# RuanJohn/Mava

Measured on AMD Instinct MI355X. Metric: env-steps/sec (whole node), ff_mappo RWARE tiny-4ag, higher is better.
Workload: dtype f32 via 2 x f16 split operands on the MFMA (3 products, f32 accumulate); 1 GPU; ff_mappo RWARE tiny-4ag-shaped synthetic obs, 4096 envs/GPU (update_batch_size=1 x num_envs=4096), rollout_length=128, ppo_epochs=4, num_minibatches=2, agents=4, obs=70/264, actions=5, one step = one PPO update = 524288 env-steps per GPU; parallelism=dp1

## Files before the change

### include/mava_hip.h

```cpp
#ifndef MAVA_HIP_H
#define MAVA_HIP_H

#include <stddef.h>
#include <stdint.h>

#ifdef __cplusplus
extern "C" {
#endif

typedef struct ihipStream_t* mava_stream_t;

const char* mava_last_error(void);
int mava_abi_version(void);

typedef struct mava_ctx mava_ctx;
enum {
  MAVA_CTX_MATMUL_MODE = 0,
  MAVA_CTX_CRITIC_AGGREGATION = 1,
  MAVA_CTX_GAE_VARIANT = 2,
  MAVA_CTX_POLICY_VARIANT = 3,
  MAVA_CTX_H2_LAUNCHES = 4,
  MAVA_CTX_TRAIN_VARIANT = 5,
  MAVA_CTX_W8_LAUNCHES = 6,
  MAVA_CTX_W1_SPLIT_FRESH = 7
};
int mava_ctx_create(mava_ctx** out);
int mava_ctx_destroy(mava_ctx* ctx);
int mava_ctx_set(mava_ctx* ctx, int key, long value);
int mava_ctx_get(const mava_ctx* ctx, int key, long* value);

int mava_gae_f32(const mava_ctx* ctx, const float* reward, const float* value, const uint8_t* done,
                 const float* last_val, const uint8_t* last_done, int T, int N, float gamma,
                 float lambda, float* adv, float* tgt, mava_stream_t s);

int mava_permutation_i32(long n, uint64_t seed, uint64_t counter, int32_t* out, mava_stream_t s);

int mava_clip_adam(float* p, const float* g, float* m, float* v, int32_t* count,
                   const int* seg_off, const float* seg_lr, int n_seg, float grad_scale,
                   float max_norm, int decay, int steps_per_update, int num_updates, float b1,
// ... 244 lines not shown
```

### mava_amd/_lib.py

```python
from __future__ import annotations

import ctypes as C
import os
from typing import Optional

import torch

_HERE = os.path.dirname(os.path.abspath(__file__))
LIB_PATH = os.environ.get("MAVA_LIB_PATH") or os.path.join(_HERE, "libmavahip.so")

_lib: Optional[C.CDLL] = None


class MavaHipError(RuntimeError):
    pass


vp = C.c_void_p
i32 = C.c_int
u32 = C.c_uint32
u64 = C.c_uint64
f32 = C.c_float
lng = C.c_long

# ... 83 lines not shown
                f"{LIB_PATH} is missing: build it with `python -m mava_amd.build` "
                "(hipcc --offload-arch=gfx950). There is no CPU fallback."
            )
        _lib = C.CDLL(LIB_PATH)
        _lib.mava_last_error.restype = C.c_char_p
        _lib.mava_last_error.argtypes = []
        for name, args in _SIGNATURES.items():
            fn = getattr(_lib, name)
            fn.argtypes = args
            fn.restype = _RESTYPES.get(name, C.c_int)
    return _lib


class Ctx:

    MATMUL_MODE, CRITIC_AGGREGATION, GAE_VARIANT, POLICY_VARIANT, H2_LAUNCHES, TRAIN_VARIANT, W8_LAUNCHES, W1_SPLIT_FRESH = 0, 1, 2, 3, 4, 5, 6, 7

    def __init__(self, matmul_mode: str = "f32", critic_aggregation: bool = True):
        if matmul_mode not in ("f32", "f16x2"):
            raise ValueError(f"matmul_mode must be 'f16x2' or 'f32', got {matmul_mode!r}")
        h = C.c_void_p()
        check(lib().mava_ctx_create(C.byref(h)), "mava_ctx_create")
        self.handle: Optional[int] = h.value
        self.set(self.MATMUL_MODE, 1 if matmul_mode == "f16x2" else 0)
        self.set(self.CRITIC_AGGREGATION, int(bool(critic_aggregation)))

    def set(self, key: int, value: int) -> None:
        check(lib().mava_ctx_set(self.handle, key, int(value)), "mava_ctx_set")

    def get(self, key: int) -> int:
        out = C.c_long()
# ... 59 lines not shown
```

### mava_amd/csrc/api.cpp

```cpp
#include <stdarg.h>
#include <stdio.h>
#include <string.h>

#include "common.h"
#include "ctx.h"

static thread_local char g_err[512] = "";

void mava_set_error(const char* fmt, ...) {
  va_list ap;
  va_start(ap, fmt);
  vsnprintf(g_err, sizeof(g_err), fmt, ap);
  va_end(ap);
}

extern "C" const char* mava_last_error(void) { return g_err; }

extern "C" int mava_abi_version(void) { return 3; }

enum { CTX_MATMUL_MODE = 0, CTX_CRITIC_AGGREGATION = 1, CTX_GAE_VARIANT = 2, CTX_POLICY_VARIANT = 3, CTX_H2_LAUNCHES = 4, CTX_TRAIN_VARIANT = 5, CTX_W8_LAUNCHES = 6, CTX_W1_SPLIT_FRESH = 7 };

extern "C" int mava_ctx_create(mava_ctx** out) {
  MAVA_ARG_CHECK(out != nullptr, 0, "mava_ctx_create: null output pointer");
  mava_ctx* c = new mava_ctx();
  c->matmul_mode = 0;
  c->critic_aggregation = 1;
  c->gae_variant = 0;
  c->policy_variant = 0;
  c->h2_launches = 0;
  c->train_variant = 0;
  c->w8_launches = 0;
  c->w1_split[0] = c->w1_split[1] = nullptr;
  for (int i = 0; i < 2; ++i) {
    c->w1_fresh[i] = 0;
    c->w1_key_params[i] = nullptr;
    c->w1_key_din[i] = c->w1_key_steps[i] = 0;
  }
  *out = c;
  return MAVA_OK;
}

extern "C" int mava_ctx_destroy(mava_ctx* c) {
  if (c == nullptr) return MAVA_OK;
  for (int i = 0; i < 2; ++i)
    if (c->w1_split[i] != nullptr) (void)hipFree(c->w1_split[i]);
  delete c;
// ... 6 lines not shown
    case CTX_MATMUL_MODE:
      MAVA_ARG_CHECK(value == 0 || value == 1, 1, "mava_ctx_set: matmul mode %ld (0 = exact f32, 1 = f16x2)", value);
      c->matmul_mode = (int)value;
      c->w1_fresh[0] = c->w1_fresh[1] = 0;
      return MAVA_OK;
    case CTX_CRITIC_AGGREGATION: c->critic_aggregation = value ? 1 : 0; return MAVA_OK;
    case CTX_GAE_VARIANT: c->gae_variant = (int)value; return MAVA_OK;
    case CTX_POLICY_VARIANT: c->policy_variant = (int)value; return MAVA_OK;
    case CTX_H2_LAUNCHES: c->h2_launches = value; return MAVA_OK;
    case CTX_TRAIN_VARIANT: c->train_variant = (int)value; return MAVA_OK;
    case CTX_W8_LAUNCHES: c->w8_launches = value; return MAVA_OK;
    case CTX_W1_SPLIT_FRESH:
      MAVA_ARG_CHECK(value == 0, 1, "mava_ctx_set: MAVA_CTX_W1_SPLIT_FRESH can only be cleared (0) by the caller");
      c->w1_fresh[0] = c->w1_fresh[1] = 0;
      return MAVA_OK;
    default: mava_set_error("mava_ctx_set: unknown key %d", key); return MAVA_EARG(2);
  }
}

extern "C" int mava_ctx_get(const mava_ctx* c, int key, long* value) {
  MAVA_ARG_CHECK(c != nullptr && value != nullptr, 0, "mava_ctx_get: null argument");
  switch (key) {
    case CTX_MATMUL_MODE: *value = c->matmul_mode; return MAVA_OK;
    case CTX_CRITIC_AGGREGATION: *value = c->critic_aggregation; return MAVA_OK;
    case CTX_GAE_VARIANT: *value = c->gae_variant; return MAVA_OK;
    case CTX_POLICY_VARIANT: *value = c->policy_variant; return MAVA_OK;
    case CTX_H2_LAUNCHES: *value = c->h2_launches; return MAVA_OK;
    case CTX_TRAIN_VARIANT: *value = c->train_variant; return MAVA_OK;
    case CTX_W8_LAUNCHES: *value = c->w8_launches; return MAVA_OK;
    case CTX_W1_SPLIT_FRESH: *value = c->w1_fresh[1]; return MAVA_OK;
    default: mava_set_error("mava_ctx_get: unknown key %d", key); return MAVA_EARG(2);
  }
}
```

### mava_amd/csrc/ctx.h

```cpp
#pragma once
#include "common.h"

struct mava_ctx {
  int matmul_mode;
  int critic_aggregation;
  int gae_variant;
  int policy_variant;
  int train_variant;
  long h2_launches;
  long w8_launches;
  void* w1_split[2];
  int w1_fresh[2];
  const float* w1_key_params[2];
  int w1_key_din[2];
  int w1_key_steps[2];
};

static inline int mava_ctx_matmul_mode(const mava_ctx* c) { return c ? c->matmul_mode : 0; }
static inline int mava_ctx_critic_aggregation(const mava_ctx* c) { return c ? c->critic_aggregation : 1; }
static inline int mava_ctx_gae_variant(const mava_ctx* c) { return c ? c->gae_variant : 0; }
static inline int mava_ctx_policy_variant(const mava_ctx* c) { return c ? c->policy_variant : 0; }
```

### mava_amd/csrc/ppo_train_h2.hip

```cpp
#include "h2_core.h"
#include "ppo_train_task.h"
#include "ctx.h"

#ifndef MAVA_GW_DEPTH
#define MAVA_GW_DEPTH 0
#endif
#define GW_DEPTH MAVA_GW_DEPTH
#ifndef MAVA_GW_DEPTH_WIDE
#define MAVA_GW_DEPTH_WIDE 0
#endif

namespace {

using namespace h2;

constexpr int STATS_BLOCKS = 128;

#ifdef MAVA_STAMPS
#define STAMP_DECL unsigned long long st_prev = __builtin_readcyclecounter(), st_acc[16] = {0, 0, 0, 0, 0, 0, 0, 0, 0, 0, 0, 0, 0, 0, 0, 0};
#define STAMP(i)                                                    \
  do {                                                              \
    __builtin_amdgcn_sched_barrier(0);                              \
    const unsigned long long st_now = __builtin_readcyclecounter(); \
    st_acc[i] += st_now - st_prev;                                  \
// ... 940 lines not shown
    if (tk.action_f != nullptr) return 1;
    if (tk.no <= 8) return dispatch_s1<8, true>(ctx, tk, n_slab, s);
#ifndef MAVA_FAST_BUILD
    if (tk.no <= 16) return dispatch_s1<16, true>(ctx, tk, n_slab, s);
    return dispatch_s1<32, true>(ctx, tk, n_slab, s);
#else
    return 1;
#endif
  }
  return dispatch_s1<1, false>(ctx, tk, n_slab, s);
}

int mava_train_h2_launch(mava_ctx* ctx, const TrainTask& tk_in, int n_slab, bool actor, hipStream_t s) {
  TrainTask tk = tk_in;
  tk.force_xlo = (ctx->train_variant & 2) != 0;
  if ((ctx->train_variant & 1) == 0) {
    const int rc8 = mava_train_w8_launch(tk, n_slab, actor, s);
    if (rc8 <= 0) {
      if (rc8 == 0) { ++ctx->h2_launches; ++ctx->w8_launches; }
      return rc8;
    }
  }
  const int rc = h2_dispatch(ctx, tk, n_slab, actor, s);
  if (rc == 0) ++ctx->h2_launches;
  return rc;
}
```

### mava_amd/csrc/ppo_train_task.h

```cpp
#pragma once
#include <stdint.h>

#include "common.h"

struct TrainTask {
  const float* params;
  const float* x;
  int din, no, xshare, xv;
  int A;
  int agg;
  const int32_t* idx;
  long idx_base;
  int Rb;
  const uint8_t* mask;
  const int32_t* action;
  const float* action_f;
  uint32_t seed_lo, seed_hi, ent_step, row_offset;
  float min_scale;
  const float* old_logp;
  const float* adv;
  const double* stats;
  const float* old_value;
  const float* targets;
  float clip_eps, ent_coef, vf_coef;
  float* slab;
  long slab_stride;
  unsigned long long* stamps;
  int force_xlo;
};

struct mava_ctx;
int mava_train_w8_launch(const TrainTask& tk, int n_slab, bool actor, hipStream_t s);
int mava_train_h2_launch(mava_ctx* ctx, const TrainTask& tk, int n_slab, bool actor, hipStream_t s);

extern int g_train_last_instance;
constexpr int train_instance_id(int family, bool actor, bool cont, bool wide, int no, int k, int xv) {
  return family * 1000000 + ((actor ? 1 : 0) + (cont ? 2 : 0) + (wide ? 4 : 0)) * 100000 + no * 1000 + k * 10 + xv;
}
```

### mava_amd/csrc/ppo_train_w8.hip

```cpp
#include "h2_core.h"
#include "ppo_train_task.h"
#include "ctx.h"

namespace {

using namespace h2;
typedef float f32x4 __attribute__((ext_vector_type(4)));

constexpr int STATS_BLOCKS = 128;
#ifndef MAVA_W8_GWD
#define MAVA_W8_GWD 1
#endif
constexpr int GWD = MAVA_W8_GWD;

#ifdef MAVA_STAMPS
#define WSTAMP_DECL unsigned long long ws_prev = __builtin_readcyclecounter(), ws_acc[16] = {0, 0, 0, 0, 0, 0, 0, 0, 0, 0, 0, 0, 0, 0, 0, 0};
#define WSTAMP(i)                                                   \
  do {                                                              \
    __builtin_amdgcn_sched_barrier(0);                              \
    const unsigned long long ws_now = __builtin_readcyclecounter(); \
    ws_acc[i] += ws_now - ws_prev;                                  \
    ws_prev = ws_now;                                               \
    __builtin_amdgcn_sched_barrier(0);                              \
  } while (0)
// ... 23 lines not shown
  c = __builtin_amdgcn_mfma_f32_16x16x16f16(a.hi, b.lo, c, 0, 0, 0);
  return __builtin_amdgcn_mfma_f32_16x16x16f16(a.hi, b.hi, c, 0, 0, 0);
}
__device__ __forceinline__ Frag4 split4(const f32x4& v) {
  Frag4 f;
#pragma unroll
  for (int r = 0; r < 4; ++r) {
    _Float16 a, b;
    split1(v[r], a, b);
    f.hi[r] = a;
    f.lo[r] = b;
  }
  return f;
}

constexpr int WROW = 256;
constexpr int WPLANE32 = 32 * WROW;
constexpr int WIMG = 2 * WPLANE32;
constexpr int W2PLANE = 128 * WROW;
constexpr int DYROW = 48;
constexpr int DYPLANE = 32 * DYROW;
__host__ __device__ inline int w8_sw(int row) { return ((row & 3) << 1) | (((row >> 3) & 1) * 9); }
__host__ __device__ inline int w8_off(int row, int chunk) { return WROW * row + 16 * (chunk ^ w8_sw(row)); }

struct W8Layout {
  int h1, dz2, dz1, w2, xs, dy, small, end;
};
inline W8Layout make_w8_layout() {
  W8Layout L;
  L.h1 = 0;
  L.dz2 = L.h1 + WIMG;
  L.dz1 = L.dz2 + WIMG;
  L.w2 = L.dz1 + WIMG;
  L.xs = L.w2 + 2 * W2PLANE;
  L.dy = L.xs + 2 * WIMG;
  L.small = L.dy + 2 * DYPLANE;
  L.end = L.small + (32 + 16 + 16) * 4;
  return L;
}

template <int NO, int S1, int XV, int W2R, bool ACTOR, int ROLE>
__device__ __forceinline__ void w8_body(const TrainTask& tk, const W8Layout& L, u8* lds) {
  constexpr bool DO_LOSS = ROLE != 2, DO_STAGE = ROLE != 1;
  constexpr float WS = ACTOR ? 1.0f : W_SCALE_CRITIC, WU = 1.0f / WS;
  constexpr int KT1 = 2 * S1;
  u8* const H1I = lds + L.h1;
  u8* const DZ2I = lds + L.dz2;
  u8* const DZ1I = lds + L.dz1;
  u8* const W2I = lds + L.w2;
  u8* const DYI = lds + L.dy;
  float* const YP = reinterpret_cast<float*>(lds + L.dz2);
  constexpr int YSTR = (NO == 8) ? 9 : NO;
  float* const B3s = reinterpret_cast<float*>(lds + L.small);
  float* const misc = B3s + 32;
  unsigned* const xflag = reinterpret_cast<unsigned*>(misc + 2);

// ... 188 lines not shown
      cursor_gather(cs, ps_next, as_next);
      stage_issue(stage_row(ps_next, as_next), xr);
    }
    if constexpr (DO_LOSS) {
      cursor_gather(cl, pl_next, al_next);
      load_row((uint32_t)pl_next * Au + al_next, r_act, r_f0, r_f1, r_m);
    }
    if constexpr (DO_STAGE) {
      stage_commit(0, xr);
      cursor_advance(cs);
    }
    if constexpr (DO_LOSS) cursor_advance(cl);
    if (it + gridDim.x < ntiles) {
      if constexpr (DO_STAGE) { cursor_gather(cs, ps_next, as_next); cursor_advance(cs); }
      if constexpr (DO_LOSS) { cursor_gather(cl, pl_next, al_next); cursor_advance(cl); }
    }
  }
  __syncthreads();

  const int swi = w8_sw(i);
  int rdA[4];
#pragma unroll
  for (int s = 0; s < 4; ++s) rdA[s] = WROW * i + 16 * ((4 * s + kg) ^ swi);
  const int wrA = WROW * i + 16 * ((2 * v + (kg >> 1)) ^ swi) + 8 * (kg & 1);
  const int tq = i >> 2, tp = i & 3;
  const int trow = 8 * kg + tq;
  const int trb = WROW * trow + 8 * (tp & 1);
  const int thx = 16 * ((tp >> 1) ^ w8_sw(trow));
  int trA[8];
#pragma unroll
// ... 2 lines not shown
    asm volatile("" : "+v"(trA[t]));
  }
  auto tr_addr = [&](int t) -> int { return trA[t]; };
  const int trOwn = tr_addr(v);
  auto read_tr = [&](const u8* img, int plane, int a0) -> Frag {
    Frag f;
    f.hi = read_tr8(img + a0, WROW);
    f.lo = read_tr8(img + plane + a0, WROW);
    return f;
  };
  auto read_row = [&](const u8* img, int plane, int a0) -> Frag { return read_row_frag(img, plane, a0); };
  const int dyRd = DYROW * i + 8 * kg;
  const int dyTr = DYROW * trow + 8 * tp;
  int buf = 0;

  WSTAMP_DECL
  for (; it < ntiles; it += gridDim.x, buf ^= 1) {
    WSTAMP(14);
    const long itn = it + gridDim.x;
    const bool have_next = itn < ntiles;
    const u8* const XSI = lds + L.xs + buf * WIMG;
    uint32_t xrow_next = DO_STAGE ? stage_row(ps_next, as_next) : 0u, lrow_next = DO_LOSS ? ((uint32_t)pl_next * Au + al_next) : 0u;
    if constexpr (DO_STAGE) asm volatile("" : "+v"(xrow_next));
    if constexpr (DO_LOSS) asm volatile("" : "+v"(lrow_next));

    f32x4 acc[2] = {f32x4{0, 0, 0, 0}, f32x4{0, 0, 0, 0}};
    const bool x_lo = __builtin_amdgcn_readfirstlane((int)xflag[buf]) != 0 || tk.force_xlo != 0;
    if (x_lo) {
      Frag xb[2];
#pragma unroll
      for (int nt = 0; nt < 2; ++nt) xb[nt] = read_row(XSI + 4096 * nt, WPLANE32, rdA[0]);
#pragma unroll
      for (int s = 0; s < S1; ++s) {
        Frag b[2] = {xb[0], xb[1]};
        if (s + 1 < S1) {
#pragma unroll
          for (int nt = 0; nt < 2; ++nt) xb[nt] = read_row(XSI + 4096 * nt, WPLANE32, rdA[(s + 1) & 3]);
        }
#pragma unroll
        for (int nt = 0; nt < 2; ++nt) acc[nt] = mfma3w(W1f[s], b[nt], acc[nt]);
        __builtin_amdgcn_sched_barrier(0);
      }
    } else {
      half8 xb[2];
#pragma unroll
      for (int nt = 0; nt < 2; ++nt) xb[nt] = *reinterpret_cast<const half8*>(XSI + 4096 * nt + rdA[0]);
#pragma unroll
      for (int s = 0; s < S1; ++s) {
        const half8 b[2] = {xb[0], xb[1]};
        if (s + 1 < S1) {
#pragma unroll
          for (int nt = 0; nt < 2; ++nt) xb[nt] = *reinterpret_cast<const half8*>(XSI + 4096 * nt + rdA[(s + 1) & 3]);
        }
#pragma unroll
        for (int nt = 0; nt < 2; ++nt) acc[nt] = mfma2w_blo0(W1f[s], b[nt], acc[nt]);
        __builtin_amdgcn_sched_barrier(0);
      }
    }
    WSTAMP(0);
    uint32_t relu1 = 0;
#pragma unroll
    for (int nt = 0; nt < 2; ++nt) {
#pragma unroll
      for (int r = 0; r < 4; ++r) {
        acc[nt][r] = fmaxf(ACTOR ? acc[nt][r] : acc[nt][r] * WU, 0.0f);
        relu1 |= (acc[nt][r] > 0.0f) ? (1u << (4 * nt + r)) : 0u;
      }
      const Frag4 f = split4(acc[nt]);
      *reinterpret_cast<half4*>(H1I + 4096 * nt + wrA) = f.hi;
      *reinterpret_cast<half4*>(H1I + 4096 * nt + WPLANE32 + wrA) = f.lo;
    }
    WSTAMP(1);
    if (have_next) {
      if constexpr (DO_STAGE) stage_issue(xrow_next, xr);
      if constexpr (DO_LOSS) load_row(lrow_next, n_act, n_f0, n_f1, n_m);
      if (itn + gridDim.x < ntiles) {
        if constexpr (DO_STAGE) { cursor_gather(cs, ps_next, as_next); cursor_advance(cs); }
        if constexpr (DO_LOSS) { cursor_gather(cl, pl_next, al_next); cursor_advance(cl); }
      }
    }
    WSTAMP(2);
    __syncthreads();
    WSTAMP(3);
    if constexpr (DO_STAGE) {
      if (tid == (ROLE == 2 ? 256 : 0)) xflag[buf ^ 1] = 0u;
    }

    f32x4 h2[2];
#pragma unroll
    for (int nt = 0; nt < 2; ++nt) h2[nt] = f32x4{b2r[0], b2r[1], b2r[2], b2r[3]};
    {
      Frag hb[2], wn;
#pragma unroll
      for (int nt = 0; nt < 2; ++nt) hb[nt] = read_row(H1I + 4096 * nt, WPLANE32, rdA[0]);
      if constexpr (W2R < 1) wn = read_tr(W2I, W2PLANE, trOwn);
#pragma unroll
      for (int s = 0; s < 4; ++s) {
        Frag b[2] = {hb[0], hb[1]};
        const Frag a = (s < W2R) ? W2f[s < W2R ? s : 0] : wn;
// ... 13 lines not shown
    for (int nt = 0; nt < 2; ++nt) {
#pragma unroll
      for (int r = 0; r < 4; ++r) {
        h2[nt][r] = fmaxf(ACTOR ? h2[nt][r] : h2[nt][r] * WU, 0.0f);
        relu2 |= (h2[nt][r] > 0.0f) ? (1u << (4 * nt + r)) : 0u;
      }
      const Frag4 f = split4(h2[nt]);
      *reinterpret_cast<half4*>(DZ1I + 4096 * nt + wrA) = f.hi;
      *reinterpret_cast<half4*>(DZ1I + 4096 * nt + WPLANE32 + wrA) = f.lo;
      const f32x4 y = mfma3k16(W3h, f, f32x4{0, 0, 0, 0});
#pragma unroll
      for (int r = 0; r < 4; ++r) {
        if (4 * kg + r < NO) YP[(v * 32 + 16 * nt + i) * YSTR + 4 * kg + r] = y[r] * W3_UNSCALE;
      }
    }
    WSTAMP(5);
    __syncthreads();
    WSTAMP(6);

    if constexpr (DO_LOSS) {
      const float lo_c = 1.0f - tk.clip_eps, hi_c = 1.0f + tk.clip_eps;
      const bool rvalid = (it * 32 + lrow) < R;
      const float* yp = YP + lrow * YSTR + lo;
      float y = B3s[lo];
#pragma unroll
      for (int u = 0; u < 8; ++u) y += yp[u * 32 * YSTR];
      float dyo = 0.0f, pg_row = 0.0f, ent_row = 0.0f;
      if constexpr (ACTOR) {
        const bool legal = (lo < no) && (r_m != 0u);
        const float z = legal ? y : -FLT_MAX;
        auto fmax_op = [](float a, float b) { return fmaxf(a, b); };
        auto add_op = [](float a, float b) { return a + b; };
        const float mx = group_allreduce<NO>(z, fmax_op);
        const float se = group_allreduce<NO>(expf(z - mx), add_op);
        const float logp = (mx == -FLT_MAX) ? ((lo < no) ? -logf((float)no) : -FLT_MAX) : z - (mx + logf(se));
        const float pr = expf(logp);
        const float ent = group_allreduce<NO>((pr > 0.0f) ? -(pr * logp) : 0.0f, add_op);
        const int act = r_act;
        const float lp = group_allreduce<NO>((lo == act) ? logp : 0.0f, add_op);
        const float gae = (r_f1 - adv_mean) * adv_rstd;
        const float ratio = expf(lp - r_f0);
// ... 15 lines not shown
        const float ov = r_f0, tg = r_f1;
        const float diff = y - ov;
        const float vclip = ov + fminf(fmaxf(diff, -tk.clip_eps), tk.clip_eps);
        const float e1 = y - tg, e2 = vclip - tg;
        const float l1 = e1 * e1, l2 = e2 * e2;
        const bool inside = (diff >= -tk.clip_eps) && (diff <= tk.clip_eps);
        const float g1 = (l1 > l2) ? 1.0f : ((l1 == l2) ? 0.5f : 0.0f);
        const float g2 = inside ? (1.0f - g1) : 0.0f;
        dyo = (rvalid && lo == 0) ? (tk.vf_coef * (g1 * e1 + g2 * e2)) : 0.0f;
        pg_row = 0.5f * fmaxf(l1, l2);
      }
      _Float16 da, db;
      split1(dyo, da, db);
      *reinterpret_cast<_Float16*>(DYI + lrow * DYROW + 2 * lo) = da;
      *reinterpret_cast<_Float16*>(DYI + DYPLANE + lrow * DYROW + 2 * lo) = db;
      ab3 += dyo;
      if (rvalid && lo == 0) {
        loss_a += pg_row * invR;
        loss_b += ent_row * invR;
      }
      r_act = n_act; r_f0 = n_f0; r_f1 = n_f1; r_m = n_m;
    }
    if constexpr (DO_STAGE) {
      if (have_next) stage_commit(buf ^ 1, xr);
    }
    WSTAMP(7);
    __syncthreads();
    WSTAMP(8);

    {
      Frag a, b;
      a.hi = read_tr8(DYI + dyTr, DYROW);
      a.lo = read_tr8(DYI + DYPLANE + dyTr, DYROW);
      b = read_tr(DZ1I, WPLANE32, trOwn);
      gW3 = mfma3w(a, b, gW3);
    }
    f32x4 dz[2];
#pragma unroll
    for (int nt = 0; nt < 2; ++nt) {
      Frag4 b;
      b.hi = *reinterpret_cast<const half4*>(DYI + 16 * nt * DYROW + dyRd);
      b.lo = *reinterpret_cast<const half4*>(DYI + DYPLANE + 16 * nt * DYROW + dyRd);
      dz[nt] = mfma3k16(W3d, b, f32x4{0, 0, 0, 0});
// ... 11 lines not shown
      const Frag b = read_tr(DZ2I, WPLANE32, trOwn);
      Frag an[GWD];
#pragma unroll
      for (int t = 0; t < GWD; ++t) an[t] = read_tr(H1I, WPLANE32, tr_addr(t));
#pragma unroll
      for (int t = 0; t < 8; ++t) {
        const Frag a = an[t % GWD];
        if (t + GWD < 8) an[t % GWD] = read_tr(H1I, WPLANE32, tr_addr(t + GWD));
        gW2[t] = mfma3w(a, b, gW2[t]);
        __builtin_amdgcn_sched_barrier(0);
      }
    }
    WSTAMP(10);
    __syncthreads();
    WSTAMP(11);

    {
      acc[0] = f32x4{0, 0, 0, 0};
      acc[1] = f32x4{0, 0, 0, 0};
      Frag an = read_row(W2I + 4096 * v, W2PLANE, rdA[0]);
      Frag bn[2];
#pragma unroll
      for (int nt = 0; nt < 2; ++nt) bn[nt] = read_row(DZ2I + 4096 * nt, WPLANE32, rdA[0]);
#pragma unroll
      for (int s = 0; s < 4; ++s) {
        const Frag a = an;
        Frag b[2] = {bn[0], bn[1]};
        if (s + 1 < 4) {
          an = read_row(W2I + 4096 * v, W2PLANE, rdA[s + 1]);
#pragma unroll
          for (int nt = 0; nt < 2; ++nt) bn[nt] = read_row(DZ2I + 4096 * nt, WPLANE32, rdA[s + 1]);
        }
#pragma unroll
        for (int nt = 0; nt < 2; ++nt) acc[nt] = mfma3w(a, b[nt], acc[nt]);
        __builtin_amdgcn_sched_barrier(0);
      }
#pragma unroll
      for (int nt = 0; nt < 2; ++nt) {
#pragma unroll
        for (int r = 0; r < 4; ++r) acc[nt][r] = ((relu1 >> (4 * nt + r)) & 1u) ? (ACTOR ? acc[nt][r] : acc[nt][r] * WU) : 0.0f;
        const Frag4 f = split4(acc[nt]);
        *reinterpret_cast<half4*>(DZ1I + 4096 * nt + wrA) = f.hi;
        *reinterpret_cast<half4*>(DZ1I + 4096 * nt + WPLANE32 + wrA) = f.lo;
      }
    }
    WSTAMP(12);
    {
      const Frag b = read_tr(DZ1I, WPLANE32, trOwn);
      constexpr int D1 = GWD < KT1 ? GWD : KT1;
      if (x_lo) {
// ... 17 lines not shown
          if (t + D1 < KT1) an[t % D1] = read_tr8(XSI + tr_addr(t + D1), WROW);
          gW1[t] = mfma2w_alo0(a, b, gW1[t]);
          __builtin_amdgcn_sched_barrier(0);
        }
      }
    }
    WSTAMP(13);
  }
#ifdef MAVA_STAMPS
  if (tk.stamps != nullptr && blockIdx.x == 0 && l == 0) {
    for (int k = 0; k < 16; ++k) tk.stamps[v * 16 + k] = ws_acc[k];
  }
#endif

  __syncthreads();
  float* slab = tk.slab + (long)blockIdx.x * tk.slab_stride;
  const int oB2 = mlp_off_b2(din), oB3 = mlp_off_b3(din, no);
  const int Pn = mlp_param_count(din, no);
#pragma unroll
  for (int t = 0; t < KT1; ++t)
#pragma unroll
    for (int r = 0; r < 4; ++r) {
      const int k = 16 * t + 4 * kg + r;
      if (k <= din) slab[k * MLP_H + 16 * v + i] = gW1[t][r] * invR;
    }
#pragma unroll
  for (int t = 0; t < 8; ++t)
#pragma unroll
    for (int r = 0; r < 4; ++r) slab[oW2 + (16 * t + 4 * kg + r) * MLP_H + 16 * v + i] = gW2[t][r] * invR;
#pragma unroll
  for (int r = 0; r < 4; ++r) {
    float x = ab2[r];
#pragma unroll
    for (int m = 1; m < 16; m <<= 1) x += __shfl_xor(x, m, 64);
    if (i == 0) slab[oB2 + 16 * v + 4 * kg + r] = x * invR;
    const int o = 4 * kg + r;
    if (o < no) slab[oW3 + (16 * v + i) * no + o] = gW3[r] * invR;
  }
  float* red = reinterpret_cast<float*>(lds + L.h1);
  if constexpr (DO_LOSS) {
    float x = ab3;
#pragma unroll
    for (int m = NO; m < 64; m <<= 1) x += __shfl_xor(x, m, 64);
    if (l < NO) red[v * NO + l] = x;
    for (int o = 32; o > 0; o >>= 1) {
      loss_a += __shfl_down(loss_a, o, 64);
      loss_b += __shfl_down(loss_b, o, 64);
    }
    if (l == 0) { red[8 * NO + 2 * v] = loss_a; red[8 * NO + 2 * v + 1] = loss_b; }
  }
  __syncthreads();
  constexpr int LW = LOSS_THREADS / 64;
  if (tid < no) {
    float x = 0.0f;
#pragma unroll
    for (int u = 0; u < LW; ++u) x += red[u * NO + tid];
    slab[oB3 + tid] = x * invR;
  }
  if (tid == 0) {
    float a = 0.0f, b = 0.0f;
#pragma unroll
    for (int u = 0; u < LW; ++u) { a += red[8 * NO + 2 * u]; b += red[8 * NO + 2 * u + 1]; }
    slab[Pn] = a;
    slab[Pn + 1] = b;
  }
}

constexpr int w8_w2r(int no, int s1, int xv) {
#ifdef MAVA_W8_W2R
  return MAVA_W8_W2R;
#else
  return (no == 8) ? ((s1 <= 2) ? 2 : ((s1 == 3 && xv == 2) ? 2 : 0)) : ((s1 <= 2) ? 2 : 0);
#endif
}
template <int NO, int S1, int XV, int W2R, bool ACTOR>
__global__ __launch_bounds__(512, 2) void ppo_train_w8_kernel(TrainTask tk, W8Layout L) {
  extern __shared__ __attribute__((aligned(16))) u8 lds[];
  if constexpr (NO == 8) {
    if (threadIdx.x < 256) {
      w8_body<NO, S1, XV, W2R, ACTOR, 1>(tk, L, lds);
    } else {
      w8_body<NO, S1, XV, W2R, ACTOR, 2>(tk, L, lds);
    }
  } else {
    w8_body<NO, S1, XV, W2R, ACTOR, 0>(tk, L, lds);
  }
}

template <int NO, int S1, int XV, bool ACTOR>
int launch_w8(const TrainTask& tk, int n_slab, hipStream_t s) {
  const W8Layout L = make_w8_layout();
  static bool attr_set = false;
  if (!attr_set) {
    MAVA_HIP_CHECK(hipFuncSetAttribute((const void*)ppo_train_w8_kernel<NO, S1, XV, w8_w2r(NO, S1, XV), ACTOR>, hipFuncAttributeMaxDynamicSharedMemorySize,
                                       L.end));
    attr_set = true;
  }
  g_train_last_instance = train_instance_id(3, ACTOR, false, false, NO, S1, XV);
  hipLaunchKernelGGL((ppo_train_w8_kernel<NO, S1, XV, w8_w2r(NO, S1, XV), ACTOR>), dim3(n_slab), dim3(512), L.end, s, tk, L);
  MAVA_LAUNCH_CHECK();
  return MAVA_OK;
}

template <int NO, int S1, bool ACTOR>
int dispatch_w8_xv(const TrainTask& tk, int n_slab, hipStream_t s) {
  if (tk.din % 2 == 0 && ((uintptr_t)tk.x) % 8 == 0) return launch_w8<NO, S1, 2, ACTOR>(tk, n_slab, s);
  if constexpr (S1 == 4) return 1;
  else return launch_w8<NO, S1, 1, ACTOR>(tk, n_slab, s);
}

template <int NO, bool ACTOR>
int dispatch_w8(const TrainTask& tk, int n_slab, hipStream_t s) {
  const int s1 = (tk.din + 1 + 31) / 32;
  switch (s1) {
#ifndef MAVA_FAST_BUILD
    case 1: return dispatch_w8_xv<NO, 1, ACTOR>(tk, n_slab, s);
    case 2: return dispatch_w8_xv<NO, 2, ACTOR>(tk, n_slab, s);
    case 4: return dispatch_w8_xv<NO, 4, ACTOR>(tk, n_slab, s);
#endif
    case 3: return dispatch_w8_xv<NO, 3, ACTOR>(tk, n_slab, s);
    default: return 1;
  }
}

}

int mava_train_w8_launch(const TrainTask& tk, int n_slab, bool actor, hipStream_t s) {
  if (tk.action_f != nullptr || tk.din + 1 > 128) return 1;
  if (!actor) {
    if (tk.agg > 1 || tk.no != 1) return 1;
    return dispatch_w8<8, false>(tk, n_slab, s);
  }
  if (tk.no <= 8) return dispatch_w8<8, true>(tk, n_slab, s);
#ifndef MAVA_FAST_BUILD
  if (tk.no <= 16) return dispatch_w8<16, true>(tk, n_slab, s);
#endif
  return 1;
}
```

Measured before the change: 74.00 million env-steps/s.

## Software-pipeline layer-1 forward of next tile into current tile's loss and backward

Adds a pipelined variant of the w8 PPO train kernel that computes the next tile's first-layer products, ReLU mask and hidden image during the current tile's loss phase and dh1 backward MFMA loop. It uses sched_group_barrier to interleave the MFMA and VALU work, and moves x staging one tile earlier (issue two tiles ahead, commit after the forward). The aim is to hide MFMA latency and the global-load latency of the x gather behind independent work. This raises register pressure, so the W2 register-residency setting is lowered for pipelined instances. The variant is on by default for S1<=2 or S1==3 with NO==8, and can be turned off through a train_variant bit.

```diff
diff --git a/include/mava_hip.h b/include/mava_hip.h
--- a/include/mava_hip.h
+++ b/include/mava_hip.h
@@ -22,7 +22,8 @@
   MAVA_CTX_H2_LAUNCHES = 4,
   MAVA_CTX_TRAIN_VARIANT = 5,
   MAVA_CTX_W8_LAUNCHES = 6,
-  MAVA_CTX_W1_SPLIT_FRESH = 7
+  MAVA_CTX_W1_SPLIT_FRESH = 7,
+  MAVA_CTX_W8_PIPELINED = 8
 };
 int mava_ctx_create(mava_ctx** out);
 int mava_ctx_destroy(mava_ctx* ctx);
diff --git a/mava_amd/_lib.py b/mava_amd/_lib.py
--- a/mava_amd/_lib.py
+++ b/mava_amd/_lib.py
@@ -121,7 +121,7 @@
 
 class Ctx:
 
-    MATMUL_MODE, CRITIC_AGGREGATION, GAE_VARIANT, POLICY_VARIANT, H2_LAUNCHES, TRAIN_VARIANT, W8_LAUNCHES, W1_SPLIT_FRESH = 0, 1, 2, 3, 4, 5, 6, 7
+    MATMUL_MODE, CRITIC_AGGREGATION, GAE_VARIANT, POLICY_VARIANT, H2_LAUNCHES, TRAIN_VARIANT, W8_LAUNCHES, W1_SPLIT_FRESH, W8_PIPELINED = 0, 1, 2, 3, 4, 5, 6, 7, 8
 
     def __init__(self, matmul_mode: str = "f32", critic_aggregation: bool = True):
         if matmul_mode not in ("f32", "f16x2"):
diff --git a/mava_amd/csrc/api.cpp b/mava_amd/csrc/api.cpp
--- a/mava_amd/csrc/api.cpp
+++ b/mava_amd/csrc/api.cpp
@@ -18,7 +18,7 @@
 
 extern "C" int mava_abi_version(void) { return 3; }
 
-enum { CTX_MATMUL_MODE = 0, CTX_CRITIC_AGGREGATION = 1, CTX_GAE_VARIANT = 2, CTX_POLICY_VARIANT = 3, CTX_H2_LAUNCHES = 4, CTX_TRAIN_VARIANT = 5, CTX_W8_LAUNCHES = 6, CTX_W1_SPLIT_FRESH = 7 };
+enum { CTX_MATMUL_MODE = 0, CTX_CRITIC_AGGREGATION = 1, CTX_GAE_VARIANT = 2, CTX_POLICY_VARIANT = 3, CTX_H2_LAUNCHES = 4, CTX_TRAIN_VARIANT = 5, CTX_W8_LAUNCHES = 6, CTX_W1_SPLIT_FRESH = 7, CTX_W8_PIPELINED = 8 };
 
 extern "C" int mava_ctx_create(mava_ctx** out) {
   MAVA_ARG_CHECK(out != nullptr, 0, "mava_ctx_create: null output pointer");
@@ -30,6 +30,7 @@
   c->h2_launches = 0;
   c->train_variant = 0;
   c->w8_launches = 0;
+  c->w8_pipelined = 0;
   c->w1_split[0] = c->w1_split[1] = nullptr;
   for (int i = 0; i < 2; ++i) {
     c->w1_fresh[i] = 0;
@@ -66,6 +67,7 @@
       MAVA_ARG_CHECK(value == 0, 1, "mava_ctx_set: MAVA_CTX_W1_SPLIT_FRESH can only be cleared (0) by the caller");
       c->w1_fresh[0] = c->w1_fresh[1] = 0;
       return MAVA_OK;
+    case CTX_W8_PIPELINED: mava_set_error("mava_ctx_set: MAVA_CTX_W8_PIPELINED is read-only"); return MAVA_EARG(1);
     default: mava_set_error("mava_ctx_set: unknown key %d", key); return MAVA_EARG(2);
   }
 }
@@ -81,6 +83,7 @@
     case CTX_TRAIN_VARIANT: *value = c->train_variant; return MAVA_OK;
     case CTX_W8_LAUNCHES: *value = c->w8_launches; return MAVA_OK;
     case CTX_W1_SPLIT_FRESH: *value = c->w1_fresh[1]; return MAVA_OK;
+    case CTX_W8_PIPELINED: *value = c->w8_pipelined; return MAVA_OK;
     default: mava_set_error("mava_ctx_get: unknown key %d", key); return MAVA_EARG(2);
   }
 }
diff --git a/mava_amd/csrc/ctx.h b/mava_amd/csrc/ctx.h
--- a/mava_amd/csrc/ctx.h
+++ b/mava_amd/csrc/ctx.h
@@ -9,6 +9,7 @@
   int train_variant;
   long h2_launches;
   long w8_launches;
+  long w8_pipelined;
   void* w1_split[2];
   int w1_fresh[2];
   const float* w1_key_params[2];
diff --git a/mava_amd/csrc/ppo_train_h2.hip b/mava_amd/csrc/ppo_train_h2.hip
--- a/mava_amd/csrc/ppo_train_h2.hip
+++ b/mava_amd/csrc/ppo_train_h2.hip
@@ -978,10 +978,12 @@
 int mava_train_h2_launch(mava_ctx* ctx, const TrainTask& tk_in, int n_slab, bool actor, hipStream_t s) {
   TrainTask tk = tk_in;
   tk.force_xlo = (ctx->train_variant & 2) != 0;
+  tk.w8_inorder = (ctx->train_variant & 4) != 0;
   if ((ctx->train_variant & 1) == 0) {
-    const int rc8 = mava_train_w8_launch(tk, n_slab, actor, s);
+    bool pipelined = false;
+    const int rc8 = mava_train_w8_launch(tk, n_slab, actor, s, &pipelined);
     if (rc8 <= 0) {
-      if (rc8 == 0) { ++ctx->h2_launches; ++ctx->w8_launches; }
+      if (rc8 == 0) { ++ctx->h2_launches; ++ctx->w8_launches; ctx->w8_pipelined += pipelined ? 1 : 0; }
       return rc8;
     }
   }
diff --git a/mava_amd/csrc/ppo_train_task.h b/mava_amd/csrc/ppo_train_task.h
--- a/mava_amd/csrc/ppo_train_task.h
+++ b/mava_amd/csrc/ppo_train_task.h
@@ -26,11 +26,12 @@
   float* slab;
   long slab_stride;
   unsigned long long* stamps;
+  int w8_inorder;
   int force_xlo;
 };
 
 struct mava_ctx;
-int mava_train_w8_launch(const TrainTask& tk, int n_slab, bool actor, hipStream_t s);
+int mava_train_w8_launch(const TrainTask& tk, int n_slab, bool actor, hipStream_t s, bool* pipelined);
 int mava_train_h2_launch(mava_ctx* ctx, const TrainTask& tk, int n_slab, bool actor, hipStream_t s);
 
 extern int g_train_last_instance;
diff --git a/mava_amd/csrc/ppo_train_w8.hip b/mava_amd/csrc/ppo_train_w8.hip
--- a/mava_amd/csrc/ppo_train_w8.hip
+++ b/mava_amd/csrc/ppo_train_w8.hip
@@ -1,6 +1,8 @@
 #include "h2_core.h"
 #include "ppo_train_task.h"
 #include "ctx.h"
+
+#include <type_traits>
 
 namespace {
 
@@ -61,6 +63,15 @@
   return f;
 }
 
+template <int NM, int VPER>
+__device__ __forceinline__ void w8_interleave() {
+#pragma unroll
+  for (int k = 0; k < NM; ++k) {
+    __builtin_amdgcn_sched_group_barrier(0x008, 1, 0);
+    __builtin_amdgcn_sched_group_barrier(0x002, VPER, 0);
+  }
+}
+
 constexpr int WROW = 256;
 constexpr int WPLANE32 = 32 * WROW;
 constexpr int WIMG = 2 * WPLANE32;
@@ -86,7 +97,7 @@
   return L;
 }
 
-template <int NO, int S1, int XV, int W2R, bool ACTOR, int ROLE>
+template <int NO, int S1, int XV, int W2R, bool ACTOR, int ROLE, bool PIPE>
 __device__ __forceinline__ void w8_body(const TrainTask& tk, const W8Layout& L, u8* lds) {
   constexpr bool DO_LOSS = ROLE != 2, DO_STAGE = ROLE != 1;
   constexpr float WS = ACTOR ? 1.0f : W_SCALE_CRITIC, WU = 1.0f / WS;
@@ -305,6 +316,10 @@
     if (it + gridDim.x < ntiles) {
       if constexpr (DO_STAGE) { cursor_gather(cs, ps_next, as_next); cursor_advance(cs); }
       if constexpr (DO_LOSS) { cursor_gather(cl, pl_next, al_next); cursor_advance(cl); }
+      if constexpr (PIPE && DO_STAGE) {
+        stage_issue(stage_row(ps_next, as_next), xr);
+        if (it + 2 * (long)gridDim.x < ntiles) { cursor_gather(cs, ps_next, as_next); cursor_advance(cs); }
+      }
     }
   }
   __syncthreads();
@@ -337,75 +352,110 @@
   const int dyTr = DYROW * trow + 8 * tp;
   int buf = 0;
 
+  auto p1_products = [&](const u8* XS, auto xlo_tag, auto fence_tag, f32x4 (&a)[2]) {
+    constexpr bool XLO = decltype(xlo_tag)::value, FENCE = decltype(fence_tag)::value;
+    a[0] = f32x4{0, 0, 0, 0};
+    a[1] = f32x4{0, 0, 0, 0};
+    if constexpr (XLO) {
+      Frag xb[2];
+#pragma unroll
+      for (int nt = 0; nt < 2; ++nt) xb[nt] = read_row(XS + 4096 * nt, WPLANE32, rdA[0]);
+#pragma unroll
+      for (int s = 0; s < S1; ++s) {
+        Frag b[2] = {xb[0], xb[1]};
+        if (s + 1 < S1) {
+#pragma unroll
+          for (int nt = 0; nt < 2; ++nt) xb[nt] = read_row(XS + 4096 * nt, WPLANE32, rdA[(s + 1) & 3]);
+        }
+#pragma unroll
+        for (int nt = 0; nt < 2; ++nt) a[nt] = mfma3w(W1f[s], b[nt], a[nt]);
+        if constexpr (FENCE) __builtin_amdgcn_sched_barrier(0);
+      }
+    } else {
+      half8 xb[2];
+#pragma unroll
+      for (int nt = 0; nt < 2; ++nt) xb[nt] = *reinterpret_cast<const half8*>(XS + 4096 * nt + rdA[0]);
+#pragma unroll
+      for (int s = 0; s < S1; ++s) {
+        const half8 b[2] = {xb[0], xb[1]};
+        if (s + 1 < S1) {
+#pragma unroll
+          for (int nt = 0; nt < 2; ++nt) xb[nt] = *reinterpret_cast<const half8*>(XS + 4096 * nt + rdA[(s + 1) & 3]);
+        }
+#pragma unroll
+        for (int nt = 0; nt < 2; ++nt) a[nt] = mfma2w_blo0(W1f[s], b[nt], a[nt]);
+        if constexpr (FENCE) __builtin_amdgcn_sched_barrier(0);
+      }
+    }
+  };
+  auto p1_mask = [&](int nt, f32x4 (&a)[2], uint32_t& relu) {
+#pragma unroll
+    for (int r = 0; r < 4; ++r) {
+      a[nt][r] = fmaxf(ACTOR ? a[nt][r] : a[nt][r] * WU, 0.0f);
+      relu |= (a[nt][r] > 0.0f) ? (1u << (4 * nt + r)) : 0u;
+    }
+  };
+  auto p1_image = [&](int nt, const f32x4 (&a)[2]) {
+    const Frag4 f = split4(a[nt]);
+    *reinterpret_cast<half4*>(H1I + 4096 * nt + wrA) = f.hi;
+    *reinterpret_cast<half4*>(H1I + 4096 * nt + WPLANE32 + wrA) = f.lo;
+  };
+  auto read_xflag = [&](int b) -> bool {
+    return __builtin_amdgcn_readfirstlane((int)xflag[b]) != 0 || tk.force_xlo != 0;
+  };
+  using std::true_type;
+  using std::false_type;
+
+  f32x4 accN[2] = {f32x4{0, 0, 0, 0}, f32x4{0, 0, 0, 0}};
+  uint32_t relu1_n = 0;
+  bool x_lo_n = false;
+  if constexpr (PIPE) {
+    if (it < ntiles) {
+      x_lo_n = read_xflag(0);
+      if (x_lo_n) p1_products(lds + L.xs, true_type{}, true_type{}, accN);
+      else p1_products(lds + L.xs, false_type{}, true_type{}, accN);
+#pragma unroll
+      for (int nt = 0; nt < 2; ++nt) { p1_mask(nt, accN, relu1_n); p1_image(nt, accN); }
+    }
+  }
+
   WSTAMP_DECL
   for (; it < ntiles; it += gridDim.x, buf ^= 1) {
     WSTAMP(14);
     const long itn = it + gridDim.x;
     const bool have_next = itn < ntiles;
     const u8* const XSI = lds + L.xs + buf * WIMG;
-    uint32_t xrow_next = DO_STAGE ? stage_row(ps_next, as_next) : 0u, lrow_next = DO_LOSS ? ((uint32_t)pl_next * Au + al_next) : 0u;
-    if constexpr (DO_STAGE) asm volatile("" : "+v"(xrow_next));
+    uint32_t xrow_next = (DO_STAGE && !PIPE) ? stage_row(ps_next, as_next) : 0u, lrow_next = DO_LOSS ? ((uint32_t)pl_next * Au + al_next) : 0u;
+    if constexpr (DO_STAGE && !PIPE) asm volatile("" : "+v"(xrow_next));
     if constexpr (DO_LOSS) asm volatile("" : "+v"(lrow_next));
 
-    f32x4 acc[2] = {f32x4{0, 0, 0, 0}, f32x4{0, 0, 0, 0}};
-    const bool x_lo = __builtin_amdgcn_readfirstlane((int)xflag[buf]) != 0 || tk.force_xlo != 0;
-    if (x_lo) {
-      Frag xb[2];
-#pragma unroll
-      for (int nt = 0; nt < 2; ++nt) xb[nt] = read_row(XSI + 4096 * nt, WPLANE32, rdA[0]);
-#pragma unroll
-      for (int s = 0; s < S1; ++s) {
-        Frag b[2] = {xb[0], xb[1]};
-        if (s + 1 < S1) {
-#pragma unroll
-          for (int nt = 0; nt < 2; ++nt) xb[nt] = read_row(XSI + 4096 * nt, WPLANE32, rdA[(s + 1) & 3]);
-        }
-#pragma unroll
-        for (int nt = 0; nt < 2; ++nt) acc[nt] = mfma3w(W1f[s], b[nt], acc[nt]);
-        __builtin_amdgcn_sched_barrier(0);
-      }
+    f32x4 acc[2];
+    bool x_lo;
+    uint32_t relu1 = 0;
+    if constexpr (!PIPE) {
+      x_lo = read_xflag(buf);
+      if (x_lo) p1_products(XSI, true_type{}, true_type{}, acc);
+      else p1_products(XSI, false_type{}, true_type{}, acc);
+      WSTAMP(0);
+#pragma unroll
+      for (int nt = 0; nt < 2; ++nt) { p1_mask(nt, acc, relu1); p1_image(nt, acc); }
+      WSTAMP(1);
     } else {
-      half8 xb[2];
-#pragma unroll
-      for (int nt = 0; nt < 2; ++nt) xb[nt] = *reinterpret_cast<const half8*>(XSI + 4096 * nt + rdA[0]);
-#pragma unroll
-      for (int s = 0; s < S1; ++s) {
-        const half8 b[2] = {xb[0], xb[1]};
-        if (s + 1 < S1) {
-#pragma unroll
-          for (int nt = 0; nt < 2; ++nt) xb[nt] = *reinterpret_cast<const half8*>(XSI + 4096 * nt + rdA[(s + 1) & 3]);
-        }
-#pragma unroll
-        for (int nt = 0; nt < 2; ++nt) acc[nt] = mfma2w_blo0(W1f[s], b[nt], acc[nt]);
-        __builtin_amdgcn_sched_barrier(0);
-      }
-    }
-    WSTAMP(0);
-    uint32_t relu1 = 0;
-#pragma unroll
-    for (int nt = 0; nt < 2; ++nt) {
-#pragma unroll
-      for (int r = 0; r < 4; ++r) {
-        acc[nt][r] = fmaxf(ACTOR ? acc[nt][r] : acc[nt][r] * WU, 0.0f);
-        relu1 |= (acc[nt][r] > 0.0f) ? (1u << (4 * nt + r)) : 0u;
-      }
-      const Frag4 f = split4(acc[nt]);
-      *reinterpret_cast<half4*>(H1I + 4096 * nt + wrA) = f.hi;
-      *reinterpret_cast<half4*>(H1I + 4096 * nt + WPLANE32 + wrA) = f.lo;
-    }
-    WSTAMP(1);
+      x_lo = x_lo_n;
+      relu1 = relu1_n;
+    }
     if (have_next) {
-      if constexpr (DO_STAGE) stage_issue(xrow_next, xr);
+      if constexpr (DO_STAGE && !PIPE) stage_issue(xrow_next, xr);
       if constexpr (DO_LOSS) load_row(lrow_next, n_act, n_f0, n_f1, n_m);
       if (itn + gridDim.x < ntiles) {
-        if constexpr (DO_STAGE) { cursor_gather(cs, ps_next, as_next); cursor_advance(cs); }
+        if constexpr (DO_STAGE && !PIPE) { cursor_gather(cs, ps_next, as_next); cursor_advance(cs); }
         if constexpr (DO_LOSS) { cursor_gather(cl, pl_next, al_next); cursor_advance(cl); }
       }
     }
     WSTAMP(2);
     __syncthreads();
     WSTAMP(3);
-    if constexpr (DO_STAGE) {
+    if constexpr (DO_STAGE && !PIPE) {
       if (tid == (ROLE == 2 ? 256 : 0)) xflag[buf ^ 1] = 0u;
     }
 
@@ -449,17 +499,21 @@
         if (4 * kg + r < NO) YP[(v * 32 + 16 * nt + i) * YSTR + 4 * kg + r] = y[r] * W3_UNSCALE;
       }
     }
+    if constexpr (PIPE && DO_STAGE) {
+      if (have_next) stage_commit(buf ^ 1, xr);
+    }
     WSTAMP(5);
     __syncthreads();
     WSTAMP(6);
 
-    if constexpr (DO_LOSS) {
+    auto loss = [&](auto&& mid) {
       const float lo_c = 1.0f - tk.clip_eps, hi_c = 1.0f + tk.clip_eps;
       const bool rvalid = (it * 32 + lrow) < R;
       const float* yp = YP + lrow * YSTR + lo;
       float y = B3s[lo];
 #pragma unroll
       for (int u = 0; u < 8; ++u) y += yp[u * 32 * YSTR];
+      if constexpr (PIPE) asm volatile("" : "+v"(y));
       float dyo = 0.0f, pg_row = 0.0f, ent_row = 0.0f;
       if constexpr (ACTOR) {
         const bool legal = (lo < no) && (r_m != 0u);
@@ -505,19 +559,41 @@
       split1(dyo, da, db);
       *reinterpret_cast<_Float16*>(DYI + lrow * DYROW + 2 * lo) = da;
       *reinterpret_cast<_Float16*>(DYI + DYPLANE + lrow * DYROW + 2 * lo) = db;
+      mid();
       ab3 += dyo;
       if (rvalid && lo == 0) {
         loss_a += pg_row * invR;
         loss_b += ent_row * invR;
       }
       r_act = n_act; r_f0 = n_f0; r_f1 = n_f1; r_m = n_m;
-    }
-    if constexpr (DO_STAGE) {
-      if (have_next) stage_commit(buf ^ 1, xr);
+    };
+    if constexpr (!PIPE) {
+      if constexpr (DO_LOSS) loss([] {});
+      if constexpr (DO_STAGE) {
+        if (have_next) stage_commit(buf ^ 1, xr);
+      }
+    } else {
+      auto p3 = [&](auto xlo_tag) {
+        constexpr bool XLO = decltype(xlo_tag)::value;
+        p1_products(lds + L.xs + (buf ^ 1) * WIMG, xlo_tag, std::integral_constant<bool, !DO_LOSS>{}, accN);
+        if constexpr (DO_LOSS) loss([] { w8_interleave<S1 * 2 * (XLO ? 3 : 2), ACTOR ? (XLO ? 11 : 16) : 2>(); });
+      };
+      if (have_next) {
+        x_lo_n = read_xflag(buf ^ 1);
+        if (x_lo_n) p3(true_type{});
+        else p3(false_type{});
+      } else {
+        accN[0] = f32x4{0, 0, 0, 0};
+        accN[1] = f32x4{0, 0, 0, 0};
+        if constexpr (DO_LOSS) loss([] {});
+      }
     }
     WSTAMP(7);
     __syncthreads();
     WSTAMP(8);
+    if constexpr (PIPE && DO_STAGE) {
+      if (tid == (ROLE == 2 ? 256 : 0)) xflag[buf] = 0u;
+    }
 
     {
       Frag a, b;
@@ -559,26 +635,58 @@
     WSTAMP(10);
     __syncthreads();
     WSTAMP(11);
+    if constexpr (PIPE && DO_STAGE) {
+      if (itn + gridDim.x < ntiles) {
+        uint32_t xrow2 = stage_row(ps_next, as_next);
+        asm volatile("" : "+v"(xrow2));
+        stage_issue(xrow2, xr);
+        if (itn + 2 * (long)gridDim.x < ntiles) { cursor_gather(cs, ps_next, as_next); cursor_advance(cs); }
+      }
+    }
+    if constexpr (PIPE) WSTAMP(0);
 
     {
       acc[0] = f32x4{0, 0, 0, 0};
       acc[1] = f32x4{0, 0, 0, 0};
-      Frag an = read_row(W2I + 4096 * v, W2PLANE, rdA[0]);
-      Frag bn[2];
-#pragma unroll
-      for (int nt = 0; nt < 2; ++nt) bn[nt] = read_row(DZ2I + 4096 * nt, WPLANE32, rdA[0]);
-#pragma unroll
-      for (int s = 0; s < 4; ++s) {
-        const Frag a = an;
-        Frag b[2] = {bn[0], bn[1]};
-        if (s + 1 < 4) {
-          an = read_row(W2I + 4096 * v, W2PLANE, rdA[s + 1]);
-#pragma unroll
-          for (int nt = 0; nt < 2; ++nt) bn[nt] = read_row(DZ2I + 4096 * nt, WPLANE32, rdA[s + 1]);
+      auto dh1 = [&](auto next_tag) {
+        constexpr bool NEXT = decltype(next_tag)::value;
+        if constexpr (NEXT) relu1_n = 0;
+        constexpr bool PF = !NEXT;
+        Frag an, bn[2];
+        if constexpr (PF) {
+          an = read_row(W2I + 4096 * v, W2PLANE, rdA[0]);
+#pragma unroll
+          for (int nt = 0; nt < 2; ++nt) bn[nt] = read_row(DZ2I + 4096 * nt, WPLANE32, rdA[0]);
         }
 #pragma unroll
-        for (int nt = 0; nt < 2; ++nt) acc[nt] = mfma3w(a, b[nt], acc[nt]);
-        __builtin_amdgcn_sched_barrier(0);
+        for (int s = 0; s < 4; ++s) {
+          if constexpr (!PF) {
+            an = read_row(W2I + 4096 * v, W2PLANE, rdA[s]);
+#pragma unroll
+            for (int nt = 0; nt < 2; ++nt) bn[nt] = read_row(DZ2I + 4096 * nt, WPLANE32, rdA[s]);
+          }
+          const Frag a = an;
+          Frag b[2] = {bn[0], bn[1]};
+          if (PF && s + 1 < 4) {
+            an = read_row(W2I + 4096 * v, W2PLANE, rdA[s + 1]);
+#pragma unroll
+            for (int nt = 0; nt < 2; ++nt) bn[nt] = read_row(DZ2I + 4096 * nt, WPLANE32, rdA[s + 1]);
+          }
+#pragma unroll
+          for (int nt = 0; nt < 2; ++nt) acc[nt] = mfma3w(a, b[nt], acc[nt]);
+          if constexpr (NEXT) {
+            if (s & 1) p1_image(s >> 1, accN);
+            else p1_mask(s >> 1, accN, relu1_n);
+            w8_interleave<6, 3>();
+          }
+          __builtin_amdgcn_sched_barrier(0);
+        }
+      };
+      if constexpr (PIPE) {
+        if (have_next) dh1(true_type{});
+        else dh1(false_type{});
+      } else {
+        dh1(false_type{});
       }
 #pragma unroll
       for (int nt = 0; nt < 2; ++nt) {
@@ -626,6 +734,9 @@
 #endif
 
   __syncthreads();
+  int tid_e = threadIdx.x;
+  asm volatile("" : "+v"(tid_e));
+  const int l_e = tid_e & 63, v_e = tid_e >> 6, i_e = l_e & 15, kg_e = l_e >> 4;
   float* slab = tk.slab + (long)blockIdx.x * tk.slab_stride;
   const int oB2 = mlp_off_b2(din), oB3 = mlp_off_b3(din, no);
   const int Pn = mlp_param_count(din, no);
@@ -633,43 +744,43 @@
   for (int t = 0; t < KT1; ++t)
 #pragma unroll
     for (int r = 0; r < 4; ++r) {
-      const int k = 16 * t + 4 * kg + r;
-      if (k <= din) slab[k * MLP_H + 16 * v + i] = gW1[t][r] * invR;
+      const int k = 16 * t + 4 * kg_e + r;
+      if (k <= din) slab[k * MLP_H + 16 * v_e + i_e] = gW1[t][r] * invR;
     }
 #pragma unroll
   for (int t = 0; t < 8; ++t)
 #pragma unroll
-    for (int r = 0; r < 4; ++r) slab[oW2 + (16 * t + 4 * kg + r) * MLP_H + 16 * v + i] = gW2[t][r] * invR;
+    for (int r = 0; r < 4; ++r) slab[oW2 + (16 * t + 4 * kg_e + r) * MLP_H + 16 * v_e + i_e] = gW2[t][r] * invR;
 #pragma unroll
   for (int r = 0; r < 4; ++r) {
     float x = ab2[r];
 #pragma unroll
     for (int m = 1; m < 16; m <<= 1) x += __shfl_xor(x, m, 64);
-    if (i == 0) slab[oB2 + 16 * v + 4 * kg + r] = x * invR;
-    const int o = 4 * kg + r;
-    if (o < no) slab[oW3 + (16 * v + i) * no + o] = gW3[r] * invR;
+    if (i_e == 0) slab[oB2 + 16 * v_e + 4 * kg_e + r] = x * invR;
+    const int o = 4 * kg_e + r;
+    if (o < no) slab[oW3 + (16 * v_e + i_e) * no + o] = gW3[r] * invR;
   }
   float* red = reinterpret_cast<float*>(lds + L.h1);
   if constexpr (DO_LOSS) {
     float x = ab3;
 #pragma unroll
     for (int m = NO; m < 64; m <<= 1) x += __shfl_xor(x, m, 64);
-    if (l < NO) red[v * NO + l] = x;
+    if (l_e < NO) red[v_e * NO + l_e] = x;
     for (int o = 32; o > 0; o >>= 1) {
       loss_a += __shfl_down(loss_a, o, 64);
       loss_b += __shfl_down(loss_b, o, 64);
     }
-    if (l == 0) { red[8 * NO + 2 * v] = loss_a; red[8 * NO + 2 * v + 1] = loss_b; }
+    if (l_e == 0) { red[8 * NO + 2 * v_e] = loss_a; red[8 * NO + 2 * v_e + 1] = loss_b; }
   }
   __syncthreads();
   constexpr int LW = LOSS_THREADS / 64;
-  if (tid < no) {
+  if (tid_e < no) {
     float x = 0.0f;
 #pragma unroll
-    for (int u = 0; u < LW; ++u) x += red[u * NO + tid];
-    slab[oB3 + tid] = x * invR;
-  }
-  if (tid == 0) {
+    for (int u = 0; u < LW; ++u) x += red[u * NO + tid_e];
+    slab[oB3 + tid_e] = x * invR;
+  }
+  if (tid_e == 0) {
     float a = 0.0f, b = 0.0f;
 #pragma unroll
     for (int u = 0; u < LW; ++u) { a += red[8 * NO + 2 * u]; b += red[8 * NO + 2 * u + 1]; }
@@ -678,74 +789,95 @@
   }
 }
 
-constexpr int w8_w2r(int no, int s1, int xv) {
+constexpr int w8_w2r(int no, int s1, int xv, bool pipe) {
 #ifdef MAVA_W8_W2R
   return MAVA_W8_W2R;
 #else
-  return (no == 8) ? ((s1 <= 2) ? 2 : ((s1 == 3 && xv == 2) ? 2 : 0)) : ((s1 <= 2) ? 2 : 0);
+  const int in_order = (no == 8) ? ((s1 <= 2) ? 2 : ((s1 == 3 && xv == 2) ? 2 : 0)) : ((s1 <= 2) ? 2 : 0);
+  return pipe ? (in_order > 1 ? 1 : in_order) : in_order;
 #endif
 }
-template <int NO, int S1, int XV, int W2R, bool ACTOR>
+constexpr bool w8_pipe(int no, int s1, int xv, bool actor) {
+#ifdef MAVA_W8_PIPE
+  return MAVA_W8_PIPE != 0;
+#else
+  (void)xv; (void)actor;
+  return s1 <= 2 || (s1 == 3 && no == 8);
+#endif
+}
+template <int NO, int S1, int XV, int W2R, bool ACTOR, bool PIPE>
 __global__ __launch_bounds__(512, 2) void ppo_train_w8_kernel(TrainTask tk, W8Layout L) {
   extern __shared__ __attribute__((aligned(16))) u8 lds[];
   if constexpr (NO == 8) {
     if (threadIdx.x < 256) {
-      w8_body<NO, S1, XV, W2R, ACTOR, 1>(tk, L, lds);
+      w8_body<NO, S1, XV, W2R, ACTOR, 1, PIPE>(tk, L, lds);
     } else {
-      w8_body<NO, S1, XV, W2R, ACTOR, 2>(tk, L, lds);
+      w8_body<NO, S1, XV, W2R, ACTOR, 2, PIPE>(tk, L, lds);
     }
   } else {
-    w8_body<NO, S1, XV, W2R, ACTOR, 0>(tk, L, lds);
-  }
-}
-
-template <int NO, int S1, int XV, bool ACTOR>
+    w8_body<NO, S1, XV, W2R, ACTOR, 0, PIPE>(tk, L, lds);
+  }
+}
+
+template <int NO, int S1, int XV, bool ACTOR, bool PIPE>
 int launch_w8(const TrainTask& tk, int n_slab, hipStream_t s) {
   const W8Layout L = make_w8_layout();
   static bool attr_set = false;
   if (!attr_set) {
-    MAVA_HIP_CHECK(hipFuncSetAttribute((const void*)ppo_train_w8_kernel<NO, S1, XV, w8_w2r(NO, S1, XV), ACTOR>, hipFuncAttributeMaxDynamicSharedMemorySize,
-                                       L.end));
+    MAVA_HIP_CHECK(hipFuncSetAttribute((const void*)ppo_train_w8_kernel<NO, S1, XV, w8_w2r(NO, S1, XV, PIPE), ACTOR, PIPE>,
+                                       hipFuncAttributeMaxDynamicSharedMemorySize, L.end));
     attr_set = true;
   }
   g_train_last_instance = train_instance_id(3, ACTOR, false, false, NO, S1, XV);
-  hipLaunchKernelGGL((ppo_train_w8_kernel<NO, S1, XV, w8_w2r(NO, S1, XV), ACTOR>), dim3(n_slab), dim3(512), L.end, s, tk, L);
+  hipLaunchKernelGGL((ppo_train_w8_kernel<NO, S1, XV, w8_w2r(NO, S1, XV, PIPE), ACTOR, PIPE>), dim3(n_slab), dim3(512), L.end, s, tk, L);
   MAVA_LAUNCH_CHECK();
   return MAVA_OK;
 }
+template <int NO, int S1, int XV, bool ACTOR>
+int launch_w8_sched(const TrainTask& tk, int n_slab, hipStream_t s, bool* pipelined) {
+  if constexpr (w8_pipe(NO, S1, XV, ACTOR)) {
+    if (tk.w8_inorder == 0) {
+      *pipelined = true;
+      return launch_w8<NO, S1, XV, ACTOR, true>(tk, n_slab, s);
+    }
+  }
+  *pipelined = false;
+  return launch_w8<NO, S1, XV, ACTOR, false>(tk, n_slab, s);
+}
 
 template <int NO, int S1, bool ACTOR>
-int dispatch_w8_xv(const TrainTask& tk, int n_slab, hipStream_t s) {
-  if (tk.din % 2 == 0 && ((uintptr_t)tk.x) % 8 == 0) return launch_w8<NO, S1, 2, ACTOR>(tk, n_slab, s);
+int dispatch_w8_xv(const TrainTask& tk, int n_slab, hipStream_t s, bool* pipelined) {
+  if (tk.din % 2 == 0 && ((uintptr_t)tk.x) % 8 == 0) return launch_w8_sched<NO, S1, 2, ACTOR>(tk, n_slab, s, pipelined);
   if constexpr (S1 == 4) return 1;
-  else return launch_w8<NO, S1, 1, ACTOR>(tk, n_slab, s);
+  else return launch_w8_sched<NO, S1, 1, ACTOR>(tk, n_slab, s, pipelined);
 }
 
 template <int NO, bool ACTOR>
-int dispatch_w8(const TrainTask& tk, int n_slab, hipStream_t s) {
+int dispatch_w8(const TrainTask& tk, int n_slab, hipStream_t s, bool* pipelined) {
   const int s1 = (tk.din + 1 + 31) / 32;
   switch (s1) {
 #ifndef MAVA_FAST_BUILD
-    case 1: return dispatch_w8_xv<NO, 1, ACTOR>(tk, n_slab, s);
-    case 2: return dispatch_w8_xv<NO, 2, ACTOR>(tk, n_slab, s);
-    case 4: return dispatch_w8_xv<NO, 4, ACTOR>(tk, n_slab, s);
+    case 1: return dispatch_w8_xv<NO, 1, ACTOR>(tk, n_slab, s, pipelined);
+    case 2: return dispatch_w8_xv<NO, 2, ACTOR>(tk, n_slab, s, pipelined);
+    case 4: return dispatch_w8_xv<NO, 4, ACTOR>(tk, n_slab, s, pipelined);
 #endif
-    case 3: return dispatch_w8_xv<NO, 3, ACTOR>(tk, n_slab, s);
+    case 3: return dispatch_w8_xv<NO, 3, ACTOR>(tk, n_slab, s, pipelined);
     default: return 1;
   }
 }
 
 }
 
-int mava_train_w8_launch(const TrainTask& tk, int n_slab, bool actor, hipStream_t s) {
+int mava_train_w8_launch(const TrainTask& tk, int n_slab, bool actor, hipStream_t s, bool* pipelined) {
+  *pipelined = false;
   if (tk.action_f != nullptr || tk.din + 1 > 128) return 1;
   if (!actor) {
     if (tk.agg > 1 || tk.no != 1) return 1;
-    return dispatch_w8<8, false>(tk, n_slab, s);
-  }
-  if (tk.no <= 8) return dispatch_w8<8, true>(tk, n_slab, s);
+    return dispatch_w8<8, false>(tk, n_slab, s, pipelined);
+  }
+  if (tk.no <= 8) return dispatch_w8<8, true>(tk, n_slab, s, pipelined);
 #ifndef MAVA_FAST_BUILD
-  if (tk.no <= 16) return dispatch_w8<16, true>(tk, n_slab, s);
+  if (tk.no <= 16) return dispatch_w8<16, true>(tk, n_slab, s, pipelined);
 #endif
   return 1;
 }
```

Result: slower. 69.47 million env-steps/s (-6.1%).
